# damien911224/ZeroShotVideoClassification

Measured on AMD Instinct MI355X. Metric: clips/sec (fwd+bwd+step) R(2+1)D-18 16x112x112 bs=22/GPU, higher is better.
Workload: dtype f32

## Files before the change

### zeroshotvideoclassification_amd/csrc/conv_wino.hip

```cpp
#include <hip/hip_runtime.h>
#include <stdlib.h>

#include "conv_params.h"
#include "zsv_common.h"
#include "zsv_hip.h"
#include "knobs.h"
#include "pack_bodies.h"

namespace zsv {

typedef __attribute__((address_space(3))) void* lds_ptr_t;
typedef float f32x2 __attribute__((ext_vector_type(2)));
typedef unsigned u32x4 __attribute__((ext_vector_type(4)));

struct WinoParams {
    int M, Mp;
    int C, nblk;
    int S, HW, W, H, T;
    int kT, R;
    int P;
    Magic m_S, m_HW, m_W, m_TH, m_H, m_tiles_m, m_ksplit;
    int wv_log2;
    int Wv, Pv;
    unsigned in_bytes, u_bytes;
// ... 587 lines not shown
                }
                const int soff = (16 * i + r) * row_bytes;
                if (!VW || nvalid >= 4) {
                    __builtin_amdgcn_raw_buffer_store_b128(__builtin_bit_cast(u32x4, y), orsrc, (int)(live ? voff + (unsigned)soff : OOBS), 0, 0);
                } else {
#pragma unroll
                    for (int e = 0; e < 3; ++e)
                        __builtin_amdgcn_raw_buffer_store_b32(__float_as_uint(y[e]), orsrc, (int)(e < nvalid ? voff + 4u * e : OOBS), soff, 0);
                }
            }
        }
        if constexpr (STATS) {
            __syncthreads();
            if (tid < BM && m0 + tid < prm.M) {
                const float t1 = (red[tid * 2] + red[(BM + tid) * 2]) + (red[(2 * BM + tid) * 2] + red[(3 * BM + tid) * 2]);
                const float t2 = (red[tid * 2 + 1] + red[(BM + tid) * 2 + 1]) + (red[(2 * BM + tid) * 2 + 1] + red[(3 * BM + tid) * 2 + 1]);
                const int tn = n0 / BN;
                prm.stat_sum[(size_t)(m0 + tid) * prm.tiles_n + tn] = t1;
                prm.stat_sq[(size_t)(m0 + tid) * prm.tiles_n + tn] = t2;
            }
        }
    } else {
    const bool stats = prm.stat_sum != nullptr;
    float* red = pool;
    if (stats) __syncthreads();
    const int quad_off = n_clip * prm.M * prm.S + sp_first;
#pragma unroll
    for (int i = 0; i < TM; ++i) {
#pragma unroll
        for (int r = 0; r < 4; ++r) {
            const int m = m0 + 16 * i + 4 * g + r;
            const float M0 = acc[0][i][r], M1 = acc[1][i][r], M2 = acc[2][i][r], M3 = acc[3][i][r], M4 = acc[4][i][r], M5 = acc[5][i][r];
            const float s12 = M1 + M2, d12 = M1 - M2, s34 = M3 + M4, d34 = M3 - M4;
            f32x4 y = {(M0 + s12) + s34, __fmaf_rn(2.f, d34, d12), __fmaf_rn(4.f, s34, s12), __fmaf_rn(8.f, d34, d12) + M5};
            float s1 = 0.f, s2 = 0.f;
            if (quad_ok && m < prm.M) {
                const int off = quad_off + m * prm.S;
                if (!VW || nvalid >= 4) {
                    s1 = (y[0] + y[1]) + (y[2] + y[3]);
                    s2 = (y[0] * y[0] + y[1] * y[1]) + (y[2] * y[2] + y[3] * y[3]);
                    if (prm.add != nullptr) y += *reinterpret_cast<const f32x4*>(prm.add + off);
                    if (prm.bias != nullptr) y += prm.bias[m];
                    if (prm.relu) { y[0] = fmaxf(y[0], 0.f); y[1] = fmaxf(y[1], 0.f); y[2] = fmaxf(y[2], 0.f); y[3] = fmaxf(y[3], 0.f); }
                    *reinterpret_cast<f32x4*>(OUT + off) = y;
                } else {
#pragma unroll
                    for (int e = 0; e < 3; ++e) {
                        if (e < nvalid) {
                            float v = y[e];
                            s1 += v;
                            s2 += v * v;
                            if (prm.add != nullptr) v += prm.add[off + e];
                            if (prm.bias != nullptr) v += prm.bias[m];
                            if (prm.relu) v = fmaxf(v, 0.f);
                            OUT[off + e] = v;
                        }
                    }
                }
            }
            if (stats) {
#pragma unroll
                for (int o = 8; o > 0; o >>= 1) {
                    s1 += __shfl_xor(s1, o, 64);
                    s2 += __shfl_xor(s2, o, 64);
                }
                if (r16 == 0) {
                    red[(wave * BM + 16 * i + 4 * g + r) * 2] = s1;
                    red[(wave * BM + 16 * i + 4 * g + r) * 2 + 1] = s2;
                }
            }
        }
    }
    if (stats) {
        __syncthreads();
        if (tid < BM && m0 + tid < prm.M) {
            const float t1 = (red[tid * 2] + red[(BM + tid) * 2]) + (red[(2 * BM + tid) * 2] + red[(3 * BM + tid) * 2]);
            const float t2 = (red[tid * 2 + 1] + red[(BM + tid) * 2 + 1]) + (red[(2 * BM + tid) * 2 + 1] + red[(3 * BM + tid) * 2 + 1]);
            const int tn = n0 / BN;
            prm.stat_sum[(size_t)(m0 + tid) * prm.tiles_n + tn] = t1;
            prm.stat_sq[(size_t)(m0 + tid) * prm.tiles_n + tn] = t2;
        }
    }
    }
#ifdef ZSV_WINOT_TRACE
    ZSV_TRACE_MARK(4);
    asm volatile("s_waitcnt vmcnt(0)" ::: "memory");
    ZSV_TRACE_MARK(5);
    if (tid == 0) {
        unsigned long long* rec = reinterpret_cast<unsigned long long*>(OUT + (prm.out_bytes >> 2)) + (size_t)blockIdx.x * 12;
        for (int i = 0; i < 6; ++i) rec[i] = trace_t[i];
        rec[6] = (unsigned)__builtin_amdgcn_s_getreg((4 << 0) | (0 << 6) | (31 << 11));
        rec[7] = (unsigned long long)tile;
        for (int i = 0; i < 3; ++i) rec[8 + i] = trace_lap[i];
        rec[11] = (trace_lap[3] << 32) | (trace_lap[4] & 0xFFFFFFFFull);
    }
#endif
#endif
}

template <int TM, bool PRE>
__global__ __launch_bounds__(256, 2) void conv_winot_kernel(WinoParams prm, const float* __restrict__ Up,
                                                            const float* __restrict__ IN, float* __restrict__ OUT) {
#if defined(__HIP_DEVICE_COMPILE__)
    constexpr int BM = 16 * TM, BK = 16;
    constexpr int LDB = 260;
    constexpr int A_FLOATS = 4 * BM * BK, B_FLOATS = BK * LDB;
    constexpr int COEF_AT = A_FLOATS + B_FLOATS;
    constexpr int STAGE = COEF_AT + (PRE ? 256 : 0);
    constexpr unsigned OOB16 = 0xFFFFFFF0u;
    extern __shared__ __attribute__((aligned(16))) float pool[];

    const int tid = threadIdx.x, lane = tid & 63;
    const int wave = __builtin_amdgcn_readfirstlane(tid >> 6);
    const int tile = xcd_tile(gridDim.x, blockIdx.x);
    const int m0 = (tile % prm.tiles_m) * BM;
    const int ct = tile / prm.tiles_m;
    const int n_img = ct / prm.segs, pos0 = (ct - n_img * prm.segs) * prm.PW;
    const int T = prm.T, PW = prm.PW, HW = prm.HW;
    const int pq = PW >> 2;

    const __amdgpu_buffer_rsrc_t rsrc = __builtin_amdgcn_make_buffer_rsrc(const_cast<float*>(IN), 0, prm.in_bytes, 0x00020000);
    const int ch_bytes = 4 * prm.S;
    const int pf = lane / pq, pp = pos0 + 4 * (lane - pf * pq);
    const unsigned piece_off = pp < HW ? (unsigned)(4 * (n_img * prm.C * prm.S + pf * HW + pp)) : OOB16;

    constexpr int APASS = TM;
    const float* a_src[APASS];
#pragma unroll
    for (int j = 0; j < APASS; ++j) {
        const int q = wave + 4 * j, pt = q / TM, ib = q % TM, row = lane >> 2;
        const int sw = ((lane & 3) ^ (((row >> 2) & 1) << 1)) * 4;
        a_src[j] = Up + ((size_t)pt * prm.Mp + m0 + 16 * ib + row) * 16 + sw;
    }
    const size_t a_chunk_stride = (size_t)4 * BK * prm.Mp;
    const __amdgpu_buffer_rsrc_t pre_rsrc =
        __builtin_amdgcn_make_buffer_rsrc(const_cast<float*>(PRE ? prm.pre_coef : IN), 0, PRE ? 8u * (unsigned)prm.pre_pitch : 0u, 0x00020000);

    const int nchunks = prm.nblk;
    auto issue = [&](int chunk, int buf) {
        float* as = pool + buf * STAGE;
        float* bs = as + A_FLOATS;
        const int ci0 = chunk * 16;
#pragma unroll
        for (int j = 0; j < 4; ++j) {
            const int k = 4 * wave + j, ci = ci0 + k;
            __builtin_amdgcn_raw_ptr_buffer_load_lds(rsrc, (lds_ptr_t)(bs + k * LDB), 16, (int)(ci < prm.C ? piece_off : OOB16),
                                                     ci < prm.C ? ci * ch_bytes : 0, 0, 0);
        }
#pragma unroll
        for (int j = 0; j < APASS; ++j)
            __builtin_amdgcn_global_load_lds(a_src[j] + (size_t)chunk * a_chunk_stride, (lds_ptr_t)(as + 256 * (wave + 4 * j)), 16, 0, 0);
        if constexpr (PRE) {
            if (wave == 0) {
                const unsigned off = lane < 8 ? 4u * (unsigned)((lane >> 2) * prm.pre_pitch + ci0 + 4 * (lane & 3)) : OOB16;
                __builtin_amdgcn_raw_ptr_buffer_load_lds(pre_rsrc, (lds_ptr_t)(as + COEF_AT), 16, (int)off, 0, 0, 0);
            }
        }
    };

    f32x4 acc[4][TM][2];
#pragma unroll
    for (int p = 0; p < 4; ++p)
#pragma unroll
        for (int i = 0; i < TM; ++i)
#pragma unroll
            for (int j = 0; j < 2; ++j) acc[p][i][j] = f32x4{0.f, 0.f, 0.f, 0.f};

    const int g = lane >> 4, r16 = lane & 15;
    int col_of[2], tp_of[2];
    bool zero_d0[2], zero_d3[2];
#pragma unroll
    for (int j = 0; j < 2; ++j) {
        const int b = 2 * wave + j, groups = PW >> 4;
        tp_of[j] = b / groups;
        col_of[j] = 16 * (b - tp_of[j] * groups) + r16;
        zero_d0[j] = tp_of[j] == 0;
        zero_d3[j] = 2 * tp_of[j] + 2 >= T;
    }

    issue(0, 0);
    __syncthreads();
    for (int ch = 0; ch < nchunks; ++ch) {
        const int cur = ch & 1;
        if (ch + 1 < nchunks) issue(ch + 1, cur ^ 1);
        const float* as = pool + cur * STAGE;
        const float* bs = as + A_FLOATS;
        f32x4 a4[4][TM];
        const int a_frag = r16 * 16 + ((g ^ (((r16 >> 2) & 1) << 1)) << 2);
#pragma unroll
        for (int p = 0; p < 4; ++p)
#pragma unroll
            for (int i = 0; i < TM; ++i) a4[p][i] = *reinterpret_cast<const f32x4*>(as + (p * TM + i) * 256 + a_frag);
        float psc[PRE ? 4 : 1], psh[PRE ? 4 : 1];
        if constexpr (PRE) {
#pragma unroll
            for (int s = 0; s < 4; ++s) {
                psc[s] = as[COEF_AT + 4 * g + s];
                psh[s] = as[COEF_AT + 16 + 4 * g + s];
            }
        }
        float raw[2][2][4];
        auto fetch = [&](int s, int slot) {
            const float* row = bs + (4 * g + s) * LDB;
#pragma unroll
            for (int j = 0; j < 2; ++j) {
                const int f0 = 2 * tp_of[j] - 1;
#pragma unroll
                for (int i = 0; i < 4; ++i) {
                    const int f = min(max(f0 + i, 0), T - 1);
                    raw[slot][j][i] = row[f * PW + col_of[j]];
                }
            }
        };
        fetch(0, 0);
#pragma unroll
        for (int s = 0; s < 4; ++s) {
            const int sl = s & 1;
            float v[4][2];
#pragma unroll
            for (int j = 0; j < 2; ++j) {
                float d[4];
#pragma unroll
                for (int i = 0; i < 4; ++i) {
                    d[i] = raw[sl][j][i];
                    if constexpr (PRE) d[i] = fmaxf(__fmaf_rn(d[i], psc[s], psh[s]), 0.f);
                }
                const float d0 = zero_d0[j] ? 0.f : d[0], d3 = zero_d3[j] ? 0.f : d[3];
                v[0][j] = d0 - d[2]; v[1][j] = d[1] + d[2]; v[2][j] = d[2] - d[1]; v[3][j] = d[1] - d3;
            }
            if (s < 3) fetch(s + 1, sl ^ 1);
            __builtin_amdgcn_sched_barrier(0);
            __builtin_amdgcn_s_setprio(1);
#pragma unroll
            for (int p = 0; p < 4; ++p)
#pragma unroll
                for (int i = 0; i < TM; ++i)
#pragma unroll
                    for (int j = 0; j < 2; ++j)
                        acc[p][i][j] = __builtin_amdgcn_mfma_f32_16x16x4f32(a4[p][i][s], v[p][j], acc[p][i][j], 0, 0, 0);
            __builtin_amdgcn_s_setprio(0);
            __builtin_amdgcn_sched_barrier(0);
        }
        __syncthreads();
    }

    const bool stats = prm.stat_sum != nullptr;
    float* red = pool;
    if (stats) __syncthreads();
    int off0[2];
    bool ok[2];
#pragma unroll
    for (int j = 0; j < 2; ++j) {
        const int pos = pos0 + col_of[j];
        ok[j] = pos < HW;
        off0[j] = n_img * prm.M * prm.S + 2 * tp_of[j] * HW + pos;
    }
#pragma unroll
    for (int i = 0; i < TM; ++i) {
#pragma unroll
        for (int r = 0; r < 4; ++r) {
            const int m = m0 + 16 * i + 4 * g + r;
            const int row_off = m * prm.S;
            float s1 = 0.f, s2 = 0.f;
#pragma unroll
            for (int j = 0; j < 2; ++j) {
                const float M0 = acc[0][i][j][r], M1 = acc[1][i][j][r], M2 = acc[2][i][j][r], M3 = acc[3][i][j][r];
                float y0 = (M0 + M1) + M2, y1 = (M1 - M2) - M3;
                if (ok[j] && m < prm.M) {
                    s1 += y0 + y1;
                    s2 += y0 * y0 + y1 * y1;
                    const int off = off0[j] + row_off;
                    if (prm.add != nullptr) { y0 += prm.add[off]; y1 += prm.add[off + HW]; }
                    if (prm.bias != nullptr) { const float bv = prm.bias[m]; y0 += bv; y1 += bv; }
                    if (prm.relu) { y0 = fmaxf(y0, 0.f); y1 = fmaxf(y1, 0.f); }
                    OUT[off] = y0;
                    OUT[off + HW] = y1;
                }
            }
            if (stats) {
#pragma unroll
                for (int o = 8; o > 0; o >>= 1) {
                    s1 += __shfl_xor(s1, o, 64);
                    s2 += __shfl_xor(s2, o, 64);
                }
                if (r16 == 0) {
                    red[(wave * BM + 16 * i + 4 * g + r) * 2] = s1;
                    red[(wave * BM + 16 * i + 4 * g + r) * 2 + 1] = s2;
                }
            }
        }
    }
    if (stats) {
        __syncthreads();
        if (tid < BM && m0 + tid < prm.M) {
            const float t1 = (red[tid * 2] + red[(BM + tid) * 2]) + (red[(2 * BM + tid) * 2] + red[(3 * BM + tid) * 2]);
            const float t2 = (red[tid * 2 + 1] + red[(BM + tid) * 2 + 1]) + (red[(2 * BM + tid) * 2 + 1] + red[(3 * BM + tid) * 2 + 1]);
            prm.stat_sum[(size_t)(m0 + tid) * prm.tiles_n + ct] = t1;
            prm.stat_sq[(size_t)(m0 + tid) * prm.tiles_n + ct] = t2;
        }
    }
#endif
}

template <int TM, bool PRE, int EPI>
__global__ __launch_bounds__(256, 2) void conv_winot4_kernel(WinoParams prm, const float* __restrict__ Up,
                                                             const float* __restrict__ IN, float* __restrict__ OUT) {
#if defined(__HIP_DEVICE_COMPILE__)
    constexpr int BM = 16 * TM, BK = 16, NP = 6;
    constexpr bool USINGLE = TM >= 4;
    constexpr int LDB = 260;
    constexpr int A_FLOATS = NP * BM * BK, B_FLOATS = BK * LDB;
    constexpr int IMG = B_FLOATS + (PRE ? 256 : 0);
    constexpr int STAGE = A_FLOATS + IMG;
    constexpr unsigned OOB16 = 0xFFFFFFF0u;
    extern __shared__ __attribute__((aligned(16))) float pool[];
    auto u_of = [&](int buf) -> float* { return pool + (USINGLE ? 0 : buf * STAGE); };
    auto img_of = [&](int buf) -> float* { return pool + (USINGLE ? A_FLOATS + buf * IMG : buf * STAGE + A_FLOATS); };

    const int tid = threadIdx.x, lane = tid & 63;
#ifdef ZSV_WINOT_TRACE
    unsigned long long trace_t[6], trace_lap[5] = {0, 0, 0, 0, 0}, trace_last = 0;
#endif
    ZSV_TRACE_MARK(0);
    const int wave = __builtin_amdgcn_readfirstlane(tid >> 6);
    const int tile = xcd_tile(gridDim.x, blockIdx.x);
    const int m0 = (tile % prm.tiles_m) * BM;
    const int ct = tile / prm.tiles_m;
    const int n_img = ct / prm.segs, pos0 = (ct - n_img * prm.segs) * prm.PW;
    const int T = prm.T, PW = prm.PW, HW = prm.HW;
    const int pq_log2 = prm.pw_log2 - 2;

    const __amdgpu_buffer_rsrc_t rsrc = __builtin_amdgcn_make_buffer_rsrc(const_cast<float*>(IN), 0, prm.in_bytes, 0x00020000);
    const int ch_bytes = 4 * prm.S;
    const int pf = lane >> pq_log2, pp = pos0 + 4 * (lane - (pf << pq_log2));
    const unsigned piece_off = pp < HW ? (unsigned)(4 * (n_img * prm.C * prm.S + pf * HW + pp)) : OOB16;

    constexpr int NPIECES = NP * TM, APASS = (NPIECES + 3) / 4;
    const __amdgpu_buffer_rsrc_t rsrc_u = __builtin_amdgcn_make_buffer_rsrc(const_cast<float*>(Up), 0, prm.u_bytes, 0x00020000);
    const int u_lane_bytes = 4 * ((m0 + (lane >> 2)) * 16 + ((lane & 3) ^ ((((lane >> 2) >> 2) & 1) << 1)) * 4);
    const int u_chunk_bytes = 4 * NP * BK * prm.Mp;
    const __amdgpu_buffer_rsrc_t pre_rsrc =
        __builtin_amdgcn_make_buffer_rsrc(const_cast<float*>(PRE ? prm.pre_coef : IN), 0, PRE ? 8u * (unsigned)prm.pre_pitch : 0u, 0x00020000);

    const int nchunks = prm.nblk;
    constexpr int NDMA = 4 + APASS + (PRE ? 1 : 0);
    auto issue_piece = [&](int chunk, int buf, int j) {
        float* as = u_of(buf);
        float* bs = img_of(buf);
        const int ci0 = chunk * 16;
        if (j < 4) {
            if (ZSV_WINOT_ABLATE == 2) return;
            const int k = 4 * wave + j, ci = ci0 + k;
            __builtin_amdgcn_raw_ptr_buffer_load_lds(rsrc, (lds_ptr_t)(bs + k * LDB), 16, (int)(ci < prm.C ? piece_off : OOB16),
                                                     ci < prm.C ? ci * ch_bytes : 0, 0, 0);
        } else if (j < 4 + APASS) {
            const int q = (3 - wave) + 4 * (j - 4);
            if (q < NPIECES && ZSV_WINOT_ABLATE != 4) {
                __builtin_amdgcn_raw_ptr_buffer_load_lds(rsrc_u, (lds_ptr_t)(as + 256 * q), 16, u_lane_bytes,
                                                         chunk * u_chunk_bytes + 4 * 16 * ((q / TM) * prm.Mp + 16 * (q % TM)), 0, 0);
            }
        } else if constexpr (PRE) {
            if (wave == 0) {
                const unsigned off = lane < 8 ? 4u * (unsigned)((lane >> 2) * prm.pre_pitch + ci0 + 4 * (lane & 3)) : OOB16;
                __builtin_amdgcn_raw_ptr_buffer_load_lds(pre_rsrc, (lds_ptr_t)(bs + B_FLOATS), 16, (int)off, 0, 0, 0);
            }
        }
    };
    auto issue = [&](int chunk, int buf) {
#pragma unroll
        for (int j = 0; j < NDMA; ++j) issue_piece(chunk, buf, j);
    };

    f32x4 acc[NP][TM];
#pragma unroll
    for (int p = 0; p < NP; ++p)
#pragma unroll
        for (int i = 0; i < TM; ++i) acc[p][i] = f32x4{0.f, 0.f, 0.f, 0.f};

    const int g = lane >> 4, r16 = lane & 15;
    int tq, col;
    if (prm.pw_log2 >= 4) {
        const int groups_log2 = prm.pw_log2 - 4;
        const int tqw = wave >> groups_log2;
        tq = tqw;
        col = 16 * (wave - (tqw << groups_log2)) + r16;
    } else {
        const int q = 16 * wave + r16;
        tq = q >> prm.pw_log2;
        col = q & (PW - 1);
    }
    const bool zero_d0 = tq == 0;
    const bool zero_d5 = 4 * tq + 4 >= T;
    const int a_frag = r16 * 16 + ((g ^ (((r16 >> 2) & 1) << 1)) << 2);

    ZSV_TRACE_MARK(1);
    issue(0, 0);
    __syncthreads();
    ZSV_TRACE_MARK(2);
#ifdef ZSV_WINOT_TRACE
    trace_last = trace_t[2];
#endif
    for (int ch = 0; ch < nchunks; ++ch) {
        const int cur = ch & 1;
        const bool prefetching = ch + 1 < nchunks;
        ZSV_TRACE_LAP(3);
        const float* as = u_of(cur);
        const float* bs = img_of(cur);
        f32x4 a4[NP][TM];
#pragma unroll
        for (int p = 0; p < NP; ++p)
#pragma unroll
            for (int i = 0; i < TM; ++i) a4[p][i] = *reinterpret_cast<const f32x4*>(as + (p * TM + i) * 256 + a_frag);
        float psc[PRE ? 4 : 1], psh[PRE ? 4 : 1];
        if constexpr (PRE) {
#pragma unroll
            for (int s = 0; s < 4; ++s) {
                psc[s] = bs[B_FLOATS + 4 * g + s];
                psh[s] = bs[B_FLOATS + 16 + 4 * g + s];
            }
        }
        float raw[2][NP];
        auto fetch = [&](int s, int slot) {
            const float* row = bs + (4 * g + s) * LDB;
            const int f0 = 4 * tq - 1;
#pragma unroll
            for (int i = 0; i < NP; ++i) {
                const int f = min(max(f0 + i, 0), T - 1);
                raw[slot][i] = row[f * PW + col];
            }
        };
        fetch(0, 0);
        ZSV_TRACE_LAP(4);
        if (USINGLE) __syncthreads();
#pragma unroll
        for (int s = 0; s < 4; ++s) {
            const int sl = s & 1;
            float d[NP];
#pragma unroll
            for (int i = 0; i < NP; ++i) {
                d[i] = raw[sl][i];
                if constexpr (PRE) d[i] = fmaxf(__fmaf_rn(d[i], psc[s], psh[s]), 0.f);
            }
            const float d0 = zero_d0 ? 0.f : d[0], d1 = d[1], d2 = d[2], d3 = d[3], d4 = d[4], d5 = zero_d5 ? 0.f : d[5];
            float v[NP];
            const float t12 = d1 + d2, t34 = d3 + d4, u12 = d1 - d2, u43 = d4 - d3, u42 = d4 - d2, u31 = d3 - d1;
            v[0] = __fmaf_rn(4.f, d0, __fmaf_rn(-5.f, d2, d4));
            v[1] = __fmaf_rn(-4.f, t12, t34);
            v[2] = __fmaf_rn(4.f, u12, u43);
            v[3] = __fmaf_rn(2.f, u31, u42);
            v[4] = __fmaf_rn(-2.f, u31, u42);
            v[5] = __fmaf_rn(4.f, d1, __fmaf_rn(-5.f, d3, d5));
            if (s < 3) fetch(s + 1, sl ^ 1);
            if (s == 0) ZSV_TRACE_LAP(0);
            __builtin_amdgcn_sched_barrier(0);
            __builtin_amdgcn_s_setprio(1);
#pragma unroll
            for (int p = 0; p < NP; ++p)
#pragma unroll
                for (int i = 0; i < TM; ++i) {
                    if (ZSV_WINOT_ABLATE == 3) acc[p][i][0] += a4[p][i][s] * v[p];
                    else acc[p][i] = __builtin_amdgcn_mfma_f32_16x16x4f32(a4[p][i][s], v[p], acc[p][i], 0, 0, 0);
                    constexpr int EV = ZSV_DMA_EVERY, PER_STEP = (NP * TM) / EV;
                    static_assert(4 * PER_STEP >= NDMA, "a slot for every DMA instruction of a chunk");
                    const int idx = p * TM + i;
                    if (idx % EV == EV - 1 && idx / EV < PER_STEP && s * PER_STEP + idx / EV < NDMA && prefetching) {
                        __builtin_amdgcn_sched_barrier(0);
                        issue_piece(ch + 1, cur ^ 1, s * PER_STEP + idx / EV);
                        __builtin_amdgcn_sched_barrier(0);
                    }
                }
            __builtin_amdgcn_s_setprio(0);
            __builtin_amdgcn_sched_barrier(0);
        }
        ZSV_TRACE_LAP(1);
        __syncthreads();
        ZSV_TRACE_LAP(2);
    }

    ZSV_TRACE_MARK(3);
    const int pos = pos0 + col;
    const bool ok = pos < HW;
    float* red = pool;
    if constexpr (EPI != 2) {
        constexpr unsigned OOB = 0xFFFFFFFFu;
        const __amdgpu_buffer_rsrc_t orsrc = __builtin_amdgcn_make_buffer_rsrc(OUT, 0, prm.out_bytes, 0x00020000);
        const unsigned lane_off = ok ? 4u * (unsigned)(n_img * prm.M * prm.S + 4 * tq * HW + pos + (m0 + 4 * g) * prm.S) : OOB;
        const bool ragged = m0 + BM > prm.M;
        const int row_bytes = 4 * prm.S, frame_bytes = 4 * HW;
        if (EPI == 1) __syncthreads();
#pragma unroll
        for (int i = 0; i < TM; ++i) {
#pragma unroll
            for (int r = 0; r < 4; ++r) {
                const float M0 = acc[0][i][r], M1 = acc[1][i][r], M2 = acc[2][i][r], M3 = acc[3][i][r], M4 = acc[4][i][r], M5 = acc[5][i][r];
                const float s12 = M1 + M2, d12 = M1 - M2, s34 = M3 + M4, d34 = M3 - M4;
                const float y[4] = {(M0 + s12) + s34, __fmaf_rn(2.f, d34, d12), __fmaf_rn(4.f, s34, s12), __fmaf_rn(8.f, d34, d12) + M5};
                unsigned voff = lane_off;
                bool live = ok;
                if (ragged) {
                    live = ok && m0 + 16 * i + 4 * g + r < prm.M;
                    voff = live ? lane_off : OOB;
                }
                const int soff = (16 * i + r) * row_bytes;
#pragma unroll
                for (int f = 0; f < 4; ++f)
                    __builtin_amdgcn_raw_buffer_store_b32(__float_as_uint(y[f]), orsrc, (int)(ZSV_WINOT_ABLATE == 1 && y[f] != 123.456f ? OOB : voff),
                                                          soff + f * frame_bytes, 0);
                if constexpr (EPI == 1) {
                    float s1 = live ? (y[0] + y[1]) + (y[2] + y[3]) : 0.f;
                    float s2 = live ? (y[0] * y[0] + y[1] * y[1]) + (y[2] * y[2] + y[3] * y[3]) : 0.f;
#define ZSV_ROW16_SUM(v)                                                                                                         \
    v += __int_as_float(__builtin_amdgcn_update_dpp(0, __float_as_int(v), 0xB1, 0xf, 0xf, true));                               \
    v += __int_as_float(__builtin_amdgcn_update_dpp(0, __float_as_int(v), 0x4E, 0xf, 0xf, true));                               \
    v += __int_as_float(__builtin_amdgcn_update_dpp(0, __float_as_int(v), 0x141, 0xf, 0xf, true));                              \
    v += __int_as_float(__builtin_amdgcn_update_dpp(0, __float_as_int(v), 0x140, 0xf, 0xf, true));
                    ZSV_ROW16_SUM(s1)
                    ZSV_ROW16_SUM(s2)
#undef ZSV_ROW16_SUM
                    if (r16 == 0) *reinterpret_cast<f32x2*>(&red[(wave * BM + 16 * i + 4 * g + r) * 2]) = f32x2{s1, s2};
                }
            }
        }
    } else {
    const bool stats = prm.stat_sum != nullptr;
    if (stats) __syncthreads();
    const int off0 = n_img * prm.M * prm.S + 4 * tq * HW + pos;
#pragma unroll
    for (int i = 0; i < TM; ++i) {
#pragma unroll
        for (int r = 0; r < 4; ++r) {
            const int m = m0 + 16 * i + 4 * g + r;
            const float M0 = acc[0][i][r], M1 = acc[1][i][r], M2 = acc[2][i][r], M3 = acc[3][i][r], M4 = acc[4][i][r], M5 = acc[5][i][r];
            const float s12 = M1 + M2, d12 = M1 - M2, s34 = M3 + M4, d34 = M3 - M4;
            float y[4] = {(M0 + s12) + s34, __fmaf_rn(2.f, d34, d12), __fmaf_rn(4.f, s34, s12), __fmaf_rn(8.f, d34, d12) + M5};
            float s1 = 0.f, s2 = 0.f;
            if (ok && m < prm.M) {
                s1 = (y[0] + y[1]) + (y[2] + y[3]);
                s2 = (y[0] * y[0] + y[1] * y[1]) + (y[2] * y[2] + y[3] * y[3]);
                const int off = off0 + m * prm.S;
#pragma unroll
                for (int f = 0; f < 4; ++f) {
                    float yv = y[f];
                    if (prm.add != nullptr) yv += prm.add[off + f * HW];
                    if (prm.bias != nullptr) yv += prm.bias[m];
                    if (prm.relu) yv = fmaxf(yv, 0.f);
                    OUT[off + f * HW] = yv;
                }
            }
            if (stats) {
#pragma unroll
                for (int o = 8; o > 0; o >>= 1) {
                    s1 += __shfl_xor(s1, o, 64);
                    s2 += __shfl_xor(s2, o, 64);
                }
                if (r16 == 0) {
                    red[(wave * BM + 16 * i + 4 * g + r) * 2] = s1;
                    red[(wave * BM + 16 * i + 4 * g + r) * 2 + 1] = s2;
                }
            }
        }
    }
    }
    if (EPI == 1 || (EPI == 2 && prm.stat_sum != nullptr)) {
        __syncthreads();
        if (tid < BM && m0 + tid < prm.M) {
            const float t1 = (red[tid * 2] + red[(BM + tid) * 2]) + (red[(2 * BM + tid) * 2] + red[(3 * BM + tid) * 2]);
            const float t2 = (red[tid * 2 + 1] + red[(BM + tid) * 2 + 1]) + (red[(2 * BM + tid) * 2 + 1] + red[(3 * BM + tid) * 2 + 1]);
            prm.stat_sum[(size_t)(m0 + tid) * prm.tiles_n + ct] = t1;
            prm.stat_sq[(size_t)(m0 + tid) * prm.tiles_n + ct] = t2;
        }
    }
#ifdef ZSV_WINOT_TRACE
    ZSV_TRACE_MARK(4);
    asm volatile("s_waitcnt vmcnt(0)" ::: "memory");
    ZSV_TRACE_MARK(5);
    if (tid == 0) {
        unsigned long long* rec = reinterpret_cast<unsigned long long*>(OUT + (prm.out_bytes >> 2)) + (size_t)blockIdx.x * 12;
        for (int i = 0; i < 6; ++i) rec[i] = trace_t[i];
        rec[6] = ((unsigned long long)__builtin_amdgcn_s_getreg((20 << 0) | (0 << 6) | (31 << 11)) << 32) |
                 (unsigned)__builtin_amdgcn_s_getreg((4 << 0) | (0 << 6) | (31 << 11));
        rec[7] = (unsigned long long)tile;
        for (int i = 0; i < 3; ++i) rec[8 + i] = trace_lap[i];
        rec[11] = (trace_lap[3] << 32) | (trace_lap[4] & 0xFFFFFFFFull);
    }
#endif
#endif
}

static size_t wino_align(size_t b) { return (b + 255) & ~(size_t)255; }

static int wino_tm(int M) {
    const int p64 = (M + 63) / 64 * 64, p48 = (M + 47) / 48 * 48;
    return p48 < p64 ? 3 : 4;
}

static bool winot_geometry(const zsv_conv_desc* d, int M);

static int wino_vw_width(const zsv_conv_desc* d) {
    if (d->Wi % 4 == 0 || ZSV_KNOB(WINO_NO_VW) || ZSV_KNOB(WINO_NO_F43)) return 0;
    for (int wv = 8; wv <= 64; wv *= 2)
        if (d->Wi < wv) return d->Wi > wv - 4 && 8 * d->Wi >= 7 * wv ? wv : 0;
    return 0;
}
static int wino_vw_plan(const zsv_conv_desc* d, int M, int& tm) {
    const int wv = wino_vw_width(d);
    const long tiles_n = ((long)d->N * d->Ti * d->Hi * wv + 255) / 256;
    const int C = M == d->Cout ? d->Cin : d->Cout;
    const long nchunks = (long)((C + 15) / 16) * 3 * d->kT;
    const char* e = ZSV_KNOB(WINO_VW_MIN_WGS);
    const long min_wgs = e ? atol(e) : 256;
    double best = 0.0;
    int best_ks = 0;
    tm = 4;
    for (int t = 4; t >= 3; --t) {
        const int bm = 16 * t;
        const long tiles = ((M + bm - 1) / bm) * tiles_n;
        const double rows = (double)M / (double)(((M + bm - 1) / bm) * bm);
        for (int ks = 1; ks <= 8; ++ks) {
            if (ks > 1 && (nchunks / ks < 12 || tiles >= 512)) break;
            const long wgs = tiles * ks;
            if (wgs < min_wgs || (ks > 1 && wgs > 1024)) continue;
            const double r = (double)wgs / 512.0, rc = (double)((wgs + 511) / 512);
            const double fill = wgs <= 512 ? r : r / (r + 0.33 * (rc - r));
            const double eff = rows * fill * (1.0 - 0.03 * (ks - 1));
            if (eff > best + 1e-9) { best = eff; best_ks = ks; tm = t; }
        }
    }
    return best_ks;
}

static int wino_ksplit(const zsv_conv_desc* d, int M) {
    if (winot_geometry(d, M)) return 1;
    if (wino_vw_width(d)) { int tm; return wino_vw_plan(d, M, tm); }
    const long P = (long)d->N * d->Ti * d->Hi * d->Wi;
    const int bm = 16 * wino_tm(M), C = M == d->Cout ? d->Cin : d->Cout;
    const long tiles = ((M + bm - 1) / bm) * ((P + 255) / 256), nchunks = (long)((C + 15) / 16) * 3 * d->kT;
    const char* e = ZSV_KNOB(WINO_MIN_TILES);
    const long min_tiles = e ? atol(e) : 512;
    if (tiles >= min_tiles) return 1;
    if (ZSV_KNOB(WINO_NO_SPLITK)) return 0;
    for (long ks = 2; ks <= 4; ++ks)
        if (tiles * ks >= min_tiles && nchunks / ks >= 12) return (int)ks;
    return 0;
}

static bool winot_shape(const zsv_conv_desc* d) {
    return d->kT == 3 && d->kH == 1 && d->kW == 1 && d->sT == 1 && d->sH == 1 && d->sW == 1 && d->pT == 1 && d->pH == 0 && d->pW == 0;
}
static int winot_segs(const zsv_conv_desc* d) {
    const int PW = 256 / d->Ti;
    return (d->Hi * d->Wi + PW - 1) / PW;
}
static bool winot_geometry(const zsv_conv_desc* d, int M) {
    if (ZSV_KNOB(NO_WINO) || ZSV_KNOB(NO_WINOT) || !winot_shape(d)) return false;
    const bool t32 = d->Ti == 32 && ZSV_KNOB(WINOT_NO_F43) == nullptr && ZSV_KNOB(WINOT_NO_T32) == nullptr;
    if ((d->Ti != 4 && d->Ti != 8 && d->Ti != 16 && !t32) || (d->Hi * d->Wi) % 4 != 0 || d->Cin < 16 || d->Cout < 16) return false;
    const long P = (long)d->N * d->Ti * d->Hi * d->Wi;
    if ((long)d->Cout * P >= (1L << 29) || (long)d->Cin * P >= (1L << 29)) return false;
    const int bm = 16 * wino_tm(M);
    const long tiles = (long)((M + bm - 1) / bm) * d->N * winot_segs(d);
    const long hw = (long)d->Hi * d->Wi, covered = (long)winot_segs(d) * (256 / d->Ti);
    const char* e1 = ZSV_KNOB(WINOT_MIN_TILES);
    const char* e2 = ZSV_KNOB(WINOT_MAX_WASTE);
    const long min_tiles = e1 ? atol(e1) : 256, max_waste = e2 ? atol(e2) : 35;
    return tiles >= min_tiles && covered * 100 <= hw * (100 + max_waste);
}

static bool wino_geometry(const zsv_conv_desc* d, int M) {
    if (winot_geometry(d, M)) return true;
    if (ZSV_KNOB(NO_WINO)) return false;
    if ((d->kT != 1 && d->kT != 3) || d->kH != 3 || d->kW != 3 || d->sT != 1 || d->sH != 1 || d->sW != 1 || d->pT != d->kT / 2 ||
        d->pH != 1 || d->pW != 1)
        return false;
    if ((d->Wi % 2 != 0 && !wino_vw_width(d)) || d->Cin < 16 || d->Cout < 16) return false;
    const long P = (long)d->N * d->Ti * d->Hi * d->Wi;
    if ((P % 2 != 0 && !wino_vw_width(d)) || (long)d->Cout * P >= (1L << 29) || (long)d->Cin * P >= (1L << 29)) return false;
    return wino_ksplit(d, M) > 0;
}

bool wino_dgrad_applicable(const zsv_conv_desc* d) { return wino_geometry(d, d->Cin); }
bool wino_fwd_applicable(const zsv_conv_desc* d) { return wino_geometry(d, d->Cout) && ZSV_KNOB(NO_WINO_FWD) == nullptr; }
int wino_fwd_stat_tiles(const zsv_conv_desc* d) {
    if (winot_geometry(d, d->Cout)) return d->N * winot_segs(d);
    if (const int wv = wino_vw_width(d)) return (int)(((long)d->N * d->Ti * d->Hi * wv + 255) / 256);
    return (int)(((long)d->N * d->Ti * d->Hi * d->Wi + 255) / 256);
}

static bool wino_f43(const zsv_conv_desc* d) { return (d->Wi % 4 == 0 && ZSV_KNOB(WINO_NO_F43) == nullptr) || wino_vw_width(d) != 0; }
static int wino_tm_for(const zsv_conv_desc* d, int M) {
    int tm = wino_tm(M);
    if (!winot_geometry(d, M) && wino_vw_width(d)) wino_vw_plan(d, M, tm);
    return tm;
}
static size_t wino_bytes(const zsv_conv_desc* d, int M, int C) {
    const int bm = 16 * wino_tm_for(d, M), Mp = (M + bm - 1) / bm * bm, nblk = (C + 15) / 16;
    if (winot_shape(d)) return wino_align((size_t)nblk * 6 * 16 * Mp * sizeof(float));
    const int points = wino_f43(d) ? 6 : 4;
    return wino_align((size_t)nblk * 3 * d->kT * points * 16 * Mp * sizeof(float));
}
static size_t wino_total_bytes(const zsv_conv_desc* d, int M, int C) {
    const int ks = wino_ksplit(d, M);
    const size_t out_bytes = (size_t)d->N * M * d->Ti * d->Hi * d->Wi * sizeof(float);
    return wino_bytes(d, M, C) + (ks > 1 ? (size_t)ks * out_bytes : 0);
}
size_t wino_dgrad_workspace_bytes(const zsv_conv_desc* d) { return wino_total_bytes(d, d->Cin, d->Cout); }
size_t wino_fwd_workspace_bytes(const zsv_conv_desc* d) { return wino_total_bytes(d, d->Cout, d->Cin); }
bool wino_dgrad_fusable(const zsv_conv_desc* d) { return wino_ksplit(d, d->Cin) == 1; }
bool wino_fwd_fusable(const zsv_conv_desc* d) { return wino_ksplit(d, d->Cout) == 1; }

template <int TM, int NCHUNKS, bool X4>
static int wino_launch(const WinoParams& p, const float* up, const float* in, float* out, hipStream_t stream) {
    constexpr int LDS_BYTES = 2 * (4 * 16 * TM * 16 + 16 * 264 + 64) * 4;
    static const hipError_t attr = hipFuncSetAttribute((const void*)conv_wino_kernel<TM, NCHUNKS, X4>, hipFuncAttributeMaxDynamicSharedMemorySize, LDS_BYTES);
    if (attr != hipSuccess) return ZSV_E_LAUNCH;
    const long tiles = (long)p.tiles_m * p.tiles_n * p.ksplit;
    hipLaunchKernelGGL((conv_wino_kernel<TM, NCHUNKS, X4>), dim3((unsigned)tiles), dim3(256), LDS_BYTES, stream, p, up, in, out);
    return launch_status();
}

template <int TM, int NCHUNKS, bool VW, int EPI>
static int wino4_launch_epi(const WinoParams& p, const float* up, const float* in, float* out, hipStream_t stream) {
    constexpr int A_FLOATS = 6 * 16 * TM * 16, IMG = 16 * 272 + 64;
    constexpr int LDS_BYTES = (TM >= 4 ? A_FLOATS + 2 * IMG : 2 * (A_FLOATS + IMG)) * 4;
    static const hipError_t attr = hipFuncSetAttribute((const void*)conv_wino4_kernel<TM, NCHUNKS, VW, EPI>, hipFuncAttributeMaxDynamicSharedMemorySize, LDS_BYTES);
    if (attr != hipSuccess) return ZSV_E_LAUNCH;
    const long tiles = (long)p.tiles_m * p.tiles_n * p.ksplit;
    hipLaunchKernelGGL((conv_wino4_kernel<TM, NCHUNKS, VW, EPI>), dim3((unsigned)tiles), dim3(256), LDS_BYTES, stream, p, up, in, out);
    return launch_status();
}
template <int TM, int NCHUNKS, bool VW = false>
static int wino4_launch(const WinoParams& p, const float* up, const float* in, float* out, hipStream_t stream) {
    if (p.bias != nullptr && p.relu && p.add == nullptr && p.stat_sum == nullptr && ZSV_KNOB(WINO_GENERIC_EPILOGUE) == nullptr)
        return wino4_launch_epi<TM, NCHUNKS, VW, 8>(p, up, in, out, stream);
    if (p.bias != nullptr || p.relu || (p.add != nullptr && p.stat_sum != nullptr) || ZSV_KNOB(WINO_GENERIC_EPILOGUE))
        return wino4_launch_epi<TM, NCHUNKS, VW, 4>(p, up, in, out, stream);
    if (p.add != nullptr) return wino4_launch_epi<TM, NCHUNKS, VW, 2>(p, up, in, out, stream);
    return p.stat_sum != nullptr ? wino4_launch_epi<TM, NCHUNKS, VW, 1>(p, up, in, out, stream) : wino4_launch_epi<TM, NCHUNKS, VW, 0>(p, up, in, out, stream);
}

template <int TM, bool PRE>
static int winot_launch(const WinoParams& p, const float* up, const float* in, float* out, hipStream_t stream) {
    constexpr int LDS_BYTES = 2 * (4 * 16 * TM * 16 + 16 * 260 + (PRE ? 256 : 0)) * 4;
    static const hipError_t attr = hipFuncSetAttribute((const void*)conv_winot_kernel<TM, PRE>, hipFuncAttributeMaxDynamicSharedMemorySize, LDS_BYTES);
    if (attr != hipSuccess) return ZSV_E_LAUNCH;
    hipLaunchKernelGGL((conv_winot_kernel<TM, PRE>), dim3((unsigned)(p.tiles_m * p.tiles_n)), dim3(256), LDS_BYTES, stream, p, up, in, out);
    return launch_status();
}

template <int TM, bool PRE, int EPI>
static int winot4_launch_epi(const WinoParams& p, const float* up, const float* in, float* out, hipStream_t stream) {
    constexpr int A_FLOATS = 6 * 16 * TM * 16, IMG = 16 * 260 + (PRE ? 256 : 0);
    constexpr int LDS_BYTES = (TM >= 4 ? A_FLOATS + 2 * IMG : 2 * (A_FLOATS + IMG)) * 4;
    static const hipError_t attr = hipFuncSetAttribute((const void*)conv_winot4_kernel<TM, PRE, EPI>, hipFuncAttributeMaxDynamicSharedMemorySize, LDS_BYTES);
    if (attr != hipSuccess) return ZSV_E_LAUNCH;
    hipLaunchKernelGGL((conv_winot4_kernel<TM, PRE, EPI>), dim3((unsigned)(p.tiles_m * p.tiles_n)), dim3(256), LDS_BYTES, stream, p, up, in, out);
    return launch_status();
}
template <int TM, bool PRE>
static int winot4_launch(const WinoParams& p, const float* up, const float* in, float* out, hipStream_t stream) {
    if (p.add != nullptr || p.bias != nullptr || p.relu || ZSV_KNOB(WINOT_GENERIC_EPILOGUE)) return winot4_launch_epi<TM, PRE, 2>(p, up, in, out, stream);
    return p.stat_sum != nullptr ? winot4_launch_epi<TM, PRE, 1>(p, up, in, out, stream) : winot4_launch_epi<TM, PRE, 0>(p, up, in, out, stream);
}

static long wino_panel_elems(const WinoParams& p, bool f43) { return (long)p.nblk * p.R * (f43 ? 6 : 4) * 16 * p.Mp; }
static bool wino_panel(PanelCtx& pc, const WinoParams& p, bool f43, const float* w, long sm, long sc, int flip, size_t need, void* workspace,
                       float*& up, int& st, hipStream_t stream) {
    const long total = wino_panel_elems(p, f43);
    auto record = [&](zsv_pack_job& job, float* panel) {
        pack_job_wino(job, f43 ? 6 : 4, PackWinoArgs{p.M, p.Mp, p.C, p.nblk, p.R, flip, sm, sc}, w, panel, total);
    };
    auto pack = [&](float* panel) {
        long pb = (total + 255) / 256;
        if (pb > 4096) pb = 4096;
        hipLaunchKernelGGL(f43 ? wino4_pack_kernel : wino_pack_kernel, dim3((unsigned)pb), dim3(256), 0, stream, w, panel, p.M, p.Mp, p.C,
                           p.nblk, p.R, sm, sc, flip, total);
    };
    return panel_ready(pc, need, workspace, up, st, record, pack);
}

static int winot_run(const zsv_conv_desc* d, int M, int C, const float* in, const float* w, long sm, long sc, int flip,
                     const float* add, const float* bias, int relu, float* stat_sum, float* stat_sq, const float* pre_coef,
                     int pre_pitch, float* out,
                     void* workspace, size_t workspace_bytes, hipStream_t stream, PanelCtx& pc) {
    if (!workspace || workspace_bytes < wino_bytes(d, M, C)) return ZSV_E_WORKSPACE;
    const int tm = wino_tm(M), bm = 16 * tm;
    WinoParams p;
    p.M = M;
    p.Mp = (M + bm - 1) / bm * bm;
    p.C = C;
    p.nblk = (C + 15) / 16;
    p.S = d->Ti * d->Hi * d->Wi; p.HW = d->Hi * d->Wi; p.W = d->Wi; p.H = d->Hi; p.T = d->Ti;
    p.kT = 3; p.R = 1;
    p.P = d->N * p.S;
    p.in_bytes = 4u * (unsigned)((long)d->N * C * p.S);
    p.PW = 256 / d->Ti;
    p.pw_log2 = d->Ti == 4 ? 6 : d->Ti == 8 ? 5 : d->Ti == 16 ? 4 : 3;
    p.out_bytes = 4u * (unsigned)((long)d->N * M * p.S);
    p.segs = winot_segs(d);
    p.tiles_m = p.Mp / bm;
    p.tiles_n = d->N * p.segs;
    p.add = add; p.bias = bias; p.relu = relu; p.stat_sum = stat_sum; p.stat_sq = stat_sq;
    p.ksplit = 1; p.chunks_per_split = p.nblk; p.slab_elems = 0;
    p.pre_coef = pre_coef; p.pre_pitch = pre_pitch;
    const bool f43 = ZSV_KNOB(WINOT_NO_F43) == nullptr;
    p.u_bytes = (unsigned)(wino_panel_elems(p, f43) * sizeof(float));
    float* up;
    int pst;
    if (!wino_panel(pc, p, f43, w, sm, sc, flip, wino_bytes(d, M, C), workspace, up, pst, stream)) return pst;
    if (f43) {
        if (pre_coef) return tm == 3 ? winot4_launch<3, true>(p, up, in, out, stream) : winot4_launch<4, true>(p, up, in, out, stream);
        return tm == 3 ? winot4_launch<3, false>(p, up, in, out, stream) : winot4_launch<4, false>(p, up, in, out, stream);
    }
    if (pre_coef) return tm == 3 ? winot_launch<3, true>(p, up, in, out, stream) : winot_launch<4, true>(p, up, in, out, stream);
    return tm == 3 ? winot_launch<3, false>(p, up, in, out, stream) : winot_launch<4, false>(p, up, in, out, stream);
}

static int wino_run(const zsv_conv_desc* d, int M, int C, const float* in, const float* w, long sm, long sc, int flip,
                    const float* add, const float* bias, int relu, float* stat_sum, float* stat_sq, float* out,
                    void* workspace, size_t workspace_bytes, hipStream_t stream, PanelCtx& pc) {
    float* const final_out = out;
    if (!workspace || workspace_bytes < wino_total_bytes(d, M, C)) return ZSV_E_WORKSPACE;
    const int tm = wino_tm_for(d, M), bm = 16 * tm;
    const int ks = wino_ksplit(d, M);
    if (ks < 1) return ZSV_E_UNSUPPORTED;
    if (ks > 1 && (add != nullptr || stat_sum != nullptr)) return ZSV_E_UNSUPPORTED;
    WinoParams p;
    p.M = M;
    p.Mp = (M + bm - 1) / bm * bm;
    p.C = C;
    p.nblk = (C + 15) / 16;
    p.S = d->Ti * d->Hi * d->Wi; p.HW = d->Hi * d->Wi; p.W = d->Wi; p.H = d->Hi; p.T = d->Ti;
    p.kT = d->kT; p.R = 3 * d->kT;
    p.P = d->N * p.S;
    p.in_bytes = 4u * (unsigned)((long)d->N * C * p.S);
    p.tiles_m = p.Mp / bm;
    p.out_bytes = 4u * (unsigned)((long)d->N * M * p.S);
    p.Wv = wino_vw_width(d);
    p.wv_log2 = 0;
    while ((1 << p.wv_log2) < p.Wv) ++p.wv_log2;
    p.m_S = make_magic((unsigned)p.S); p.m_HW = make_magic((unsigned)p.HW); p.m_W = make_magic((unsigned)p.W);
    p.m_TH = make_magic((unsigned)(p.T * p.H)); p.m_H = make_magic((unsigned)p.H);
    p.m_tiles_m = make_magic((unsigned)p.tiles_m); p.m_ksplit = make_magic((unsigned)ks);
    p.Pv = p.Wv ? d->N * d->Ti * d->Hi * p.Wv : p.P;
    p.tiles_n = (p.Pv + 255) / 256;
    p.add = add; p.bias = bias; p.relu = relu; p.stat_sum = stat_sum; p.stat_sq = stat_sq;
    p.ksplit = ks;
    p.chunks_per_split = (p.nblk * p.R + ks - 1) / ks;
    p.slab_elems = (long)d->N * M * p.S;
    float* slabs = (float*)((char*)workspace + wino_bytes(d, M, C));
    if (ks > 1) { p.bias = nullptr; p.relu = 0; out = slabs; }
    const bool f43 = wino_f43(d);
    p.u_bytes = (unsigned)wino_bytes(d, M, C);
    float* up;
    int pst;
    if (!wino_panel(pc, p, f43, w, sm, sc, flip, wino_bytes(d, M, C), workspace, up, pst, stream)) return pst;
    const bool x4 = d->Wi % 4 == 0 && ZSV_KNOB(WINO_NO_X4) == nullptr;
    int st;
    if (p.Wv) {
        st = tm == 3 ? wino4_launch<3, 0, true>(p, up, in, out, stream) : wino4_launch<4, 0, true>(p, up, in, out, stream);
    } else if (f43) {
        if (tm == 3) st = (p.nblk * p.R == 12 && ks == 1) ? wino4_launch<3, 12>(p, up, in, out, stream) : wino4_launch<3, 0>(p, up, in, out, stream);
        else st = wino4_launch<4, 0>(p, up, in, out, stream);
    } else if (tm == 3) {
        if (x4) st = (p.nblk * p.R == 12 && ks == 1) ? wino_launch<3, 12, true>(p, up, in, out, stream) : wino_launch<3, 0, true>(p, up, in, out, stream);
        else st = wino_launch<3, 0, false>(p, up, in, out, stream);
    } else {
        st = x4 ? wino_launch<4, 0, true>(p, up, in, out, stream) : wino_launch<4, 0, false>(p, up, in, out, stream);
    }
    if (st || ks == 1) return st;
    return splitk_reduce(slabs, ks, p.slab_elems, M, p.S, bias, relu, final_out, stream);
}

int wino_dgrad(const zsv_conv_desc* d, const float* dy, const float* w, const float* add, float* dx, void* workspace,
               size_t workspace_bytes, hipStream_t stream, PanelCtx& pc) {
    if (winot_geometry(d, d->Cin))
        return winot_run(d, d->Cin, d->Cout, dy, w, 3, (long)d->Cin * 3, 1, add, nullptr, 0, nullptr, nullptr, nullptr, 0, dx, workspace,
                         workspace_bytes, stream, pc);
    const long taps = 9L * d->kT;
    return wino_run(d, d->Cin, d->Cout, dy, w, taps, (long)d->Cin * taps, 1, add, nullptr, 0, nullptr, nullptr, dx, workspace,
                    workspace_bytes, stream, pc);
}

bool wino_fwd_pre_capable(const zsv_conv_desc* d) { return winot_geometry(d, d->Cout) && ZSV_KNOB(NO_WINO_FWD) == nullptr; }

int wino_fwd_pre(const zsv_conv_desc* d, const float* x, const float* pre_coef, int pre_pitch, const float* w, float* stat_sum,
                 float* stat_sq, float* y, void* workspace, size_t workspace_bytes, hipStream_t stream, PanelCtx& pc) {
    if (!wino_fwd_pre_capable(d)) return ZSV_E_UNSUPPORTED;
    return winot_run(d, d->Cout, d->Cin, x, w, (long)d->Cin * 3, 3, 0, nullptr, nullptr, 0, stat_sum, stat_sq, pre_coef, pre_pitch, y, workspace,
                     workspace_bytes, stream, pc);
}

int wino_fwd(const zsv_conv_desc* d, const float* x, const float* w, const float* bias, const float* residual, int relu,
             float* stat_sum, float* stat_sq, float* y, void* workspace, size_t workspace_bytes, hipStream_t stream, PanelCtx& pc) {
    if (winot_geometry(d, d->Cout))
        return winot_run(d, d->Cout, d->Cin, x, w, (long)d->Cin * 3, 3, 0, residual, bias, relu, stat_sum, stat_sq, nullptr, 0, y,
                         workspace, workspace_bytes, stream, pc);
    const long taps = 9L * d->kT;
    return wino_run(d, d->Cout, d->Cin, x, w, (long)d->Cin * taps, taps, 0, residual, bias, relu, stat_sum, stat_sq, y, workspace,
                    workspace_bytes, stream, pc);
}

}
```

### zeroshotvideoclassification_amd/csrc/knobs.h

```cpp
#pragma once

#define ZSV_KNOB_LIST(X) \
    X(NO_FUSED_STATS) \
    X(NO_BN_FUSION) \
    X(BF16_NO_SAME) \
    X(BF16_NO_TSAME) \
    X(BF16_NO_SAME64) \
    X(BF16_NO_SAME9) \
    X(BF16_SAME9_MIN_CHUNKS) \
    X(WINOT_NO_T32) \
    X(BF16_GROUP_OUTER) \
    X(BF16_NO_WGRAD) \
    X(BF16_NO_WGRAD_GATHER) \
    X(BF16_WGRAD_WGS) \
    X(NO_DGRAD_S2) \
    X(NO_DGRAD_S2T) \
    X(DGRAD_S2_BN) \
    X(DGRAD_S2_KS) \
    X(NO_DOWN_FUSION) \
    X(DGRAD_S2_NO_X4) \
    X(CONV_CFG) \
    X(NO_SPLITK) \
    X(TAP_KS) \
    X(SPLITK_THRESH) \
    X(NO_CFG5) \
    X(NO_TAP) \
    X(NO_LDS_EPILOGUE) \
    X(WGRAD_CFG) \
    X(WGRAD_BN) \
    X(WGRAD_WGS) \
    X(WGRAD_NO_TWOTAP) \
    X(NO_WGRAD_DMA) \
    X(WGRAD_DMA_TM) \
    X(WGRAD_DMA_TN) \
    X(WGRAD_DMA_SLICES) \
    X(WGRAD_LINEAR_WALK) \
    X(NO_STEM_WGRAD) \
    X(STEM_WGRAD_WGS) \
    X(WGRAD_TRING_RESIDENT) \
    X(WGRAD_TRING_SLICES) \
    X(NO_WGRAD_TRING) \
    X(NO_WGRAD_TWINO) \
    X(WGRAD_WINO_SLICES) \
    X(NO_WINO) \
    X(NO_WGRAD_WINO) \
    X(NO_WGRAD_WINO4) \
    X(WINO_MIN_TILES) \
    X(WINO_NO_SPLITK) \
    X(NO_WINOT) \
    X(WINOT_MIN_TILES) \
    X(BN_NT_MB) \
    X(BN_NO_MASKED_G) \
    X(WINOT_MAX_WASTE) \
    X(NO_WINO_FWD) \
    X(WINO_NO_F43) \
    X(WINOT_NO_F43) \
    X(WINO_NO_X4) \
    X(NO_SLAB_SUM_ROWS) \
    X(SPLITK_REDUCE_SCALAR) \
    X(NO_PACK_TILED) \
    X(NO_T2_DENSE) \
    X(WINO_NO_VW) \
    X(WINO_VW_MIN_WGS) \
    X(WINOT_GENERIC_EPILOGUE) \
    X(WINO_GENERIC_EPILOGUE)

namespace zsv {
enum KnobId {
#define ZSV_KNOB_ENUM(name) K_##name,
    ZSV_KNOB_LIST(ZSV_KNOB_ENUM)
#undef ZSV_KNOB_ENUM
    K_COUNT
};
extern const char* volatile g_knobs[K_COUNT];
}

#define ZSV_KNOB(name) (::zsv::g_knobs[::zsv::K_##name])
```

Measured before the change: 576.0.

## Run the 48-row temporal Winograd kernel at three workgroups per CU

```diff
diff --git a/zeroshotvideoclassification_amd/csrc/conv_wino.hip b/zeroshotvideoclassification_amd/csrc/conv_wino.hip
--- a/zeroshotvideoclassification_amd/csrc/conv_wino.hip
+++ b/zeroshotvideoclassification_amd/csrc/conv_wino.hip
@@ -913,12 +913,13 @@
 #endif
 }
 
-template <int TM, bool PRE, int EPI>
-__global__ __launch_bounds__(256, 2) void conv_winot4_kernel(WinoParams prm, const float* __restrict__ Up,
-                                                             const float* __restrict__ IN, float* __restrict__ OUT) {
+template <int TM, bool PRE, int EPI, bool WG3 = false>
+__global__ __launch_bounds__(256, WG3 ? 3 : 2) void conv_winot4_kernel(WinoParams prm, const float* __restrict__ Up,
+                                                                       const float* __restrict__ IN, float* __restrict__ OUT) {
 #if defined(__HIP_DEVICE_COMPILE__)
+    static_assert(!WG3 || (TM == 3 && !PRE), "three workgroups per CU: the 48-row tile without the folded BatchNorm");
     constexpr int BM = 16 * TM, BK = 16, NP = 6;
-    constexpr bool USINGLE = TM >= 4;
+    constexpr bool USINGLE = TM >= 4 || WG3;
     constexpr int LDB = 260;
     constexpr int A_FLOATS = NP * BM * BK, B_FLOATS = BK * LDB;
     constexpr int IMG = B_FLOATS + (PRE ? 256 : 0);
@@ -1017,6 +1018,88 @@
         ZSV_TRACE_LAP(3);
         const float* as = u_of(cur);
         const float* bs = img_of(cur);
+        if constexpr (WG3) {
+        constexpr int HP = NP / 2;
+        f32x4 a4[HP][TM];
+#pragma unroll
+        for (int p = 0; p < HP; ++p)
+#pragma unroll
+            for (int i = 0; i < TM; ++i) a4[p][i] = *reinterpret_cast<const f32x4*>(as + (p * TM + i) * 256 + a_frag);
+        float raw[2][NP], vk[4][HP];
+        auto fetch = [&](int s, int slot) {
+            const float* row = bs + (4 * g + s) * LDB;
+            const int f0 = 4 * tq - 1;
+#pragma unroll
+            for (int i = 0; i < NP; ++i) {
+                const int f = min(max(f0 + i, 0), T - 1);
+                raw[slot][i] = row[f * PW + col];
+            }
+        };
+        fetch(0, 0);
+        ZSV_TRACE_LAP(4);
+#pragma unroll
+        for (int s = 0; s < 4; ++s) {
+            const int sl = s & 1;
+            const float d0 = zero_d0 ? 0.f : raw[sl][0], d1 = raw[sl][1], d2 = raw[sl][2], d3 = raw[sl][3], d4 = raw[sl][4],
+                        d5 = zero_d5 ? 0.f : raw[sl][5];
+            float v[HP];
+            const float t12 = d1 + d2, t34 = d3 + d4, u12 = d1 - d2, u43 = d4 - d3, u42 = d4 - d2, u31 = d3 - d1;
+            v[0] = __fmaf_rn(4.f, d0, __fmaf_rn(-5.f, d2, d4));
+            v[1] = __fmaf_rn(-4.f, t12, t34);
+            v[2] = __fmaf_rn(4.f, u12, u43);
+            vk[s][0] = __fmaf_rn(2.f, u31, u42);
+            vk[s][1] = __fmaf_rn(-2.f, u31, u42);
+            vk[s][2] = __fmaf_rn(4.f, d1, __fmaf_rn(-5.f, d3, d5));
+            if (s < 3) fetch(s + 1, sl ^ 1);
+            if (s == 0) ZSV_TRACE_LAP(0);
+            __builtin_amdgcn_sched_barrier(0);
+            __builtin_amdgcn_s_setprio(1);
+#pragma unroll
+            for (int p = 0; p < HP; ++p)
+#pragma unroll
+                for (int i = 0; i < TM; ++i) {
+                    acc[p][i] = __builtin_amdgcn_mfma_f32_16x16x4f32(a4[p][i][s], v[p], acc[p][i], 0, 0, 0);
+                    const int idx = p * TM + i;
+                    if (s == 3) {
+                        __builtin_amdgcn_sched_barrier(0);
+                        a4[p][i] = *reinterpret_cast<const f32x4*>(as + ((p + HP) * TM + i) * 256 + a_frag);
+                        __builtin_amdgcn_sched_barrier(0);
+                    }
+                    if (s < 2 && (idx == 2 || idx == 6) && prefetching) {
+                        __builtin_amdgcn_sched_barrier(0);
+                        issue_piece(ch + 1, cur ^ 1, 2 * s + (idx == 6 ? 1 : 0));
+                        __builtin_amdgcn_sched_barrier(0);
+                    }
+                }
+            __builtin_amdgcn_s_setprio(0);
+            __builtin_amdgcn_sched_barrier(0);
+        }
+        asm volatile("s_waitcnt lgkmcnt(0)" ::: "memory");
+        __builtin_amdgcn_s_barrier();
+        __builtin_amdgcn_sched_barrier(0);
+        __builtin_amdgcn_s_setprio(1);
+#pragma unroll
+        for (int s = 0; s < 4; ++s)
+#pragma unroll
+            for (int p = 0; p < HP; ++p)
+#pragma unroll
+                for (int i = 0; i < TM; ++i) {
+                    acc[p + HP][i] = __builtin_amdgcn_mfma_f32_16x16x4f32(a4[p][i][s], vk[s][p], acc[p + HP][i], 0, 0, 0);
+                    constexpr int EV = ZSV_DMA_EVERY;
+                    static_assert(4 * HP * TM >= EV * APASS, "a slot for every U piece of a chunk");
+                    const int n = (s * HP + p) * TM + i;
+                    if (n % EV == EV / 3 && n / EV < APASS && prefetching) {
+                        __builtin_amdgcn_sched_barrier(0);
+                        issue_piece(ch + 1, cur ^ 1, 4 + n / EV);
+                        __builtin_amdgcn_sched_barrier(0);
+                    }
+                }
+        __builtin_amdgcn_s_setprio(0);
+        __builtin_amdgcn_sched_barrier(0);
+        ZSV_TRACE_LAP(1);
+        __syncthreads();
+        ZSV_TRACE_LAP(2);
+        } else {
         f32x4 a4[NP][TM];
 #pragma unroll
         for (int p = 0; p < NP; ++p)
@@ -1086,6 +1169,7 @@
         ZSV_TRACE_LAP(1);
         __syncthreads();
         ZSV_TRACE_LAP(2);
+        }
     }
 
     ZSV_TRACE_MARK(3);
@@ -1358,19 +1442,24 @@
     return launch_status();
 }
 
-template <int TM, bool PRE, int EPI>
+template <int TM, bool PRE, int EPI, bool WG3 = false>
 static int winot4_launch_epi(const WinoParams& p, const float* up, const float* in, float* out, hipStream_t stream) {
     constexpr int A_FLOATS = 6 * 16 * TM * 16, IMG = 16 * 260 + (PRE ? 256 : 0);
-    constexpr int LDS_BYTES = (TM >= 4 ? A_FLOATS + 2 * IMG : 2 * (A_FLOATS + IMG)) * 4;
-    static const hipError_t attr = hipFuncSetAttribute((const void*)conv_winot4_kernel<TM, PRE, EPI>, hipFuncAttributeMaxDynamicSharedMemorySize, LDS_BYTES);
+    constexpr int LDS_BYTES = (TM >= 4 || WG3 ? A_FLOATS + 2 * IMG : 2 * (A_FLOATS + IMG)) * 4;
+    static_assert(!WG3 || 3 * LDS_BYTES <= 160 * 1024, "three workgroups per CU");
+    static const hipError_t attr = hipFuncSetAttribute((const void*)conv_winot4_kernel<TM, PRE, EPI, WG3>, hipFuncAttributeMaxDynamicSharedMemorySize, LDS_BYTES);
     if (attr != hipSuccess) return ZSV_E_LAUNCH;
-    hipLaunchKernelGGL((conv_winot4_kernel<TM, PRE, EPI>), dim3((unsigned)(p.tiles_m * p.tiles_n)), dim3(256), LDS_BYTES, stream, p, up, in, out);
+    hipLaunchKernelGGL((conv_winot4_kernel<TM, PRE, EPI, WG3>), dim3((unsigned)(p.tiles_m * p.tiles_n)), dim3(256), LDS_BYTES, stream, p, up, in, out);
     return launch_status();
 }
 template <int TM, bool PRE>
 static int winot4_launch(const WinoParams& p, const float* up, const float* in, float* out, hipStream_t stream) {
-    if (p.add != nullptr || p.bias != nullptr || p.relu || ZSV_KNOB(WINOT_GENERIC_EPILOGUE)) return winot4_launch_epi<TM, PRE, 2>(p, up, in, out, stream);
-    return p.stat_sum != nullptr ? winot4_launch_epi<TM, PRE, 1>(p, up, in, out, stream) : winot4_launch_epi<TM, PRE, 0>(p, up, in, out, stream);
+    constexpr bool CAN3 = TM == 3 && !PRE;
+    const bool wg3 = CAN3 && ZSV_KNOB(WINOT_NO_3WG) == nullptr;
+    if (p.add != nullptr || p.bias != nullptr || p.relu || ZSV_KNOB(WINOT_GENERIC_EPILOGUE))
+        return wg3 ? winot4_launch_epi<TM, PRE, 2, CAN3>(p, up, in, out, stream) : winot4_launch_epi<TM, PRE, 2>(p, up, in, out, stream);
+    if (p.stat_sum != nullptr) return wg3 ? winot4_launch_epi<TM, PRE, 1, CAN3>(p, up, in, out, stream) : winot4_launch_epi<TM, PRE, 1>(p, up, in, out, stream);
+    return wg3 ? winot4_launch_epi<TM, PRE, 0, CAN3>(p, up, in, out, stream) : winot4_launch_epi<TM, PRE, 0>(p, up, in, out, stream);
 }
 
 static long wino_panel_elems(const WinoParams& p, bool f43) { return (long)p.nblk * p.R * (f43 ? 6 : 4) * 16 * p.Mp; }
diff --git a/zeroshotvideoclassification_amd/csrc/knobs.h b/zeroshotvideoclassification_amd/csrc/knobs.h
--- a/zeroshotvideoclassification_amd/csrc/knobs.h
+++ b/zeroshotvideoclassification_amd/csrc/knobs.h
@@ -63,6 +63,7 @@
     X(WINO_NO_VW) \
     X(WINO_VW_MIN_WGS) \
     X(WINOT_GENERIC_EPILOGUE) \
+    X(WINOT_NO_3WG) \
     X(WINO_GENERIC_EPILOGUE)
 
 namespace zsv {
```

New measurement: 574.9. Within noise of the previous version (-0.2%).
